# undistro/trivy

Measured on AMD Instinct MI355X. Metric: GB/s secret-scanned (whole node) at 1/2/4/8 MI355X; findings bit-exact vs CPU, higher is better.
Workload: dtype u8

## Files before the change

include/tsg_debug.h:

```cpp
#ifndef TSG_DEBUG_H
#define TSG_DEBUG_H
#include <stdint.h>
#ifdef __cplusplus
extern "C" {
#endif

int tsg_regex_find_all(const char* pattern, const uint8_t* text, uint64_t n, int submatch,
                       const int64_t* windows, uint32_t n_windows, int64_t* out, uint64_t out_cap,
                       uint64_t* out_len, int32_t* num_cap);

void tsg_debug_regex_engine(int mode);
int tsg_debug_xform(int device, const uint8_t* raw, uint64_t n_bytes, const uint64_t* offsets, uint32_t n_files,
                    const uint8_t* kinds, uint8_t* out, uint64_t out_cap, uint64_t* xoff);
int tsg_debug_classify(int device, const uint8_t* raw, uint64_t n_bytes, const uint64_t* offsets, uint32_t n_files,
                       uint8_t* flags);
int tsg_debug_transform_census(int device, const uint8_t* raw, uint64_t n_bytes, const uint64_t* offsets,
                               uint32_t n_files, const uint8_t* kinds, uint8_t* mark_out);
int tsg_debug_gather_device(int device, const uint8_t* raw, uint64_t n_bytes, const uint64_t* src_off,
                            const uint64_t* dst_off, uint32_t n_files, uint8_t* out);
int tsg_regex_match(const char* pattern, const uint8_t* text, uint64_t n);

int64_t tsg_go_bytes_to_lower(const uint8_t* s, uint64_t n, uint8_t* out, uint64_t out_cap);

struct tsg_global;
typedef struct tsg_compiled tsg_compiled;
struct tsg_table_info;
typedef struct tsg_debug_rule_info {
  uint32_t nfa_words;
  uint32_t gate;
  uint32_t anchored;
  uint32_t has_regex;
  const uint64_t* nfa;
  const uint32_t* kw_ids;
  uint32_t n_kw;
} tsg_debug_rule_info;
int tsg_debug_compile(const struct tsg_global* g, tsg_compiled** out);
struct tsg_compile_options;
int tsg_debug_compile_ex(const struct tsg_global* g, const struct tsg_compile_options* opt, tsg_compiled** out,
                         uint32_t* out_calibrated);
void tsg_debug_compiled_free(tsg_compiled* c);
int tsg_debug_compiled_info(const tsg_compiled* c, struct tsg_table_info* out);
int tsg_debug_rule(const tsg_compiled* c, uint32_t i, tsg_debug_rule_info* out);
int tsg_debug_rule_gate_implied(const tsg_compiled* c, uint32_t i);
int tsg_debug_anchor(const tsg_compiled* c, uint32_t j, uint32_t* rule, uint32_t* lit_len,
                     int32_t* off_lo, int32_t* off_hi);
const char* tsg_debug_keyword(const tsg_compiled* c, uint32_t k);
const void* tsg_debug_anchor_req(const tsg_compiled* c, uint32_t j);
int tsg_debug_filter(const tsg_compiled* c, uint32_t* shape, const uint32_t** reach, const uint32_t** bucket_off,
                     const uint32_t** bucket_items, const void** items, uint32_t* n_items, const uint8_t** item_cls,
                     const uint32_t** classes, double* est_fp);
int tsg_debug_filter_ids(const tsg_compiled* c, const uint32_t** ids, uint32_t* n);
const char* tsg_debug_rule_anchor(const tsg_compiled* c, uint32_t i);


int tsg_debug_pool_budget(void);

struct tsg_scanner;
int tsg_debug_scanner_engine(struct tsg_scanner* s, uint64_t out[4]);

int tsg_debug_scanner_gpu_findings(struct tsg_scanner* s, int mode);

int tsg_debug_scanner_fetch(struct tsg_scanner* s, uint64_t stage_bytes, uint64_t direct_bytes);

int tsg_regex_find_all_bounded(const char* pattern, const uint8_t* text, uint64_t true_len, uint64_t lo, uint64_t hi,
                               int submatch, const int64_t* windows, uint32_t n_windows, int64_t* out,
                               uint64_t out_cap, uint64_t* out_len, int32_t* num_cap, int32_t* hit_limit);
int tsg_debug_fetch_windows_plan(const uint64_t* offsets, uint32_t n_files, const void* cands, uint64_t n_cands,
                                 const uint32_t* rule_max_len, uint32_t n_rules, const uint32_t* opts, uint64_t* runs,
                                 uint64_t runs_cap, uint64_t* n_runs, uint64_t* views, uint64_t views_cap,
                                 uint64_t* n_views, uint64_t totals[4]);
int tsg_debug_fetch_windows_device(int device, const uint8_t* arena, uint64_t n_bytes, const uint64_t* offsets,
                                   uint32_t n_files, const void* cands, uint64_t n_cands, uint32_t cand_cap,
                                   const uint32_t* rule_max_len, uint32_t n_rules, const uint32_t* opts,
                                   uint64_t stage_bytes, uint8_t* packed, uint64_t packed_cap, uint64_t counters[4]);

struct tsg_batch;
struct tsg_result;
struct tsg_fetch_window_stats;
int tsg_debug_sparse_tail(const struct tsg_global* g, const struct tsg_batch* batch, const void* cands,
                          uint64_t n_cands, const uint32_t* opts, struct tsg_result** out,
                          struct tsg_fetch_window_stats* window_stats);

int tsg_debug_sure_allow(const char* const* patterns, uint32_t n_patterns, const uint8_t* paths, const uint64_t* off,
                         uint32_t n_paths, uint8_t* sure, uint8_t* has_form);
int tsg_debug_result_skip(const struct tsg_result* r, uint64_t out[6]);
int tsg_debug_result_k0(const struct tsg_result* r, double* ms_k0);

typedef struct tsg_debug_stage_dump {
  uint32_t struct_size;
  uint32_t kw_words;
  uint32_t counters[16];
  uint32_t caps[3];
  uint32_t reserved_;
  uint64_t* hits;        uint64_t hits_cap, n_hits;
  uint32_t* kw;          uint64_t kw_cap, n_kw;
  uint32_t* flags;       uint64_t flags_cap, n_flags;
  uint16_t* nl;          uint64_t nl_cap, n_nl;
  uint32_t* chunk_file;  uint64_t chunk_file_cap, n_chunk_file;
  uint32_t* recs;        uint64_t recs_cap, n_recs;
  void* cands;           uint64_t cands_cap, n_cands;
} tsg_debug_stage_dump;
int tsg_debug_engine_stages(const tsg_compiled* c, int device, const uint8_t* arena, uint64_t n_bytes,
                            const uint64_t* offsets, uint32_t n_files, const uint8_t tail[64],
                            tsg_debug_stage_dump* out);

const char* tsg_last_error(void);

#ifdef __cplusplus
}
#endif
#endif
```

trivy_amd/csrc/capi_debug.cpp:

```cpp
#include "tsg_debug.h"

#include <algorithm>
#include <atomic>
#include <cstring>
#include <memory>
#include <string>
#include <vector>

#include "capi_internal.h"
#include "census.h"
#include "classify.h"
#include "fetch_host.h"
#include "fetch_windows.h"
#include "goregex.h"
#include "parallel.h"
#include "xform.h"

namespace tsg {
extern std::atomic<int> g_regex_engine;
thread_local std::string g_last_error;
void SetError(const std::string& e) { g_last_error = e; }
}

extern "C" {

const char* tsg_last_error(void) { return tsg::g_last_error.c_str(); }

int tsg_regex_find_all(const char* pattern, const uint8_t* text, uint64_t n, int submatch,
                       const int64_t* windows, uint32_t n_windows, int64_t* out, uint64_t out_cap,
                       uint64_t* out_len, int32_t* num_cap) {
  std::string err;
  auto re = tsg::Regex::Compile(pattern, &err);
  if (!re) {
    tsg::SetError(err);
    return -1;
  }
  std::vector<tsg::Window> wins;
  for (uint32_t i = 0; i < n_windows; i++) wins.push_back({windows[2 * i], windows[2 * i + 1]});
  std::vector<int64_t> res;
  re->FindAll(text, int64_t(n), submatch != 0, windows ? &wins : nullptr, &res);
  *out_len = res.size();
  *num_cap = re->num_cap();
  if (!res.empty()) std::memcpy(out, res.data(), sizeof(int64_t) * (res.size() < out_cap ? res.size() : out_cap));
  return 0;
}

void tsg_debug_regex_engine(int mode) { tsg::g_regex_engine.store(mode); }

int tsg_debug_xform(int device, const uint8_t* raw, uint64_t n_bytes, const uint64_t* offsets, uint32_t n_files,
                    const uint8_t* kinds, uint8_t* out, uint64_t out_cap, uint64_t* xoff) {
  if (offsets[0] != 0 || offsets[n_files] != n_bytes) {
    tsg::SetError("offsets must run from 0 to n_bytes");
    return -2;
  }
  void *d_raw = nullptr, *d_off = nullptr, *d_kind = nullptr, *d_xoff = nullptr, *d_out = nullptr, *d_sc = nullptr;
  hipStream_t s = nullptr;
  hipError_t e = hipSetDevice(device);
  auto ok = [&](hipError_t r) {
    if (e == hipSuccess) e = r;
    return e == hipSuccess;
  };
  const size_t sc_bytes = tsg::XformScratchBytes(n_bytes, n_files);
  if (ok(e) && ok(hipStreamCreate(&s)) && ok(hipMalloc(&d_raw, n_bytes + 64)) &&
      ok(hipMalloc(&d_off, (size_t(n_files) + 1) * 8)) && ok(hipMalloc(&d_kind, size_t(n_files) + 1)) &&
      ok(hipMalloc(&d_xoff, (size_t(n_files) + 1) * 8)) && ok(hipMalloc(&d_sc, sc_bytes)) &&
      ok(hipMemset(d_raw, 0, n_bytes + 64)) && ok(hipMemcpy(d_raw, raw, n_bytes, hipMemcpyHostToDevice)) &&
      ok(hipMemcpy(d_off, offsets, (size_t(n_files) + 1) * 8, hipMemcpyHostToDevice)) &&
      ok(hipMemcpy(d_kind, kinds, n_files, hipMemcpyHostToDevice)) && tsg::XformOnePassOn()) {
    const uint64_t cap = tsg::XformMaxOut(n_bytes, n_files) + 64;
    if (ok(hipMalloc(&d_out, cap)) &&
        ok(tsg::XformOnePass(static_cast<const uint8_t*>(d_raw), n_bytes, static_cast<const uint64_t*>(d_off),
                             static_cast<const uint8_t*>(d_kind), n_files, d_sc, static_cast<uint64_t*>(d_xoff),
                             static_cast<uint8_t*>(d_out), cap, s)) &&
        ok(hipMemcpyAsync(xoff, d_xoff, (size_t(n_files) + 1) * 8, hipMemcpyDeviceToHost, s)) &&
        ok(hipStreamSynchronize(s)) &&
        ok(tsg::XformErrorWord(n_bytes, n_files, d_sc, s) == 0 ? hipSuccess : hipErrorIllegalAddress))
      ok(hipMemcpy(out, d_out, std::min<uint64_t>(out_cap, xoff[n_files]), hipMemcpyDeviceToHost));
  } else if (ok(e) &&
      ok(tsg::XformPlan(static_cast<const uint8_t*>(d_raw), n_bytes, static_cast<const uint64_t*>(d_off),
                        static_cast<const uint8_t*>(d_kind), n_files, d_sc, static_cast<uint64_t*>(d_xoff), s)) &&
      ok(hipMemcpyAsync(xoff, d_xoff, (size_t(n_files) + 1) * 8, hipMemcpyDeviceToHost, s)) &&
      ok(hipStreamSynchronize(s)) && ok(hipMalloc(&d_out, xoff[n_files] + 64)) &&
      ok(tsg::XformWrite(static_cast<const uint8_t*>(d_raw), n_bytes, static_cast<const uint64_t*>(d_off),
                         static_cast<const uint8_t*>(d_kind), n_files, d_sc, static_cast<uint8_t*>(d_out),
                         xoff[n_files] + 64, s)) &&
      ok(hipStreamSynchronize(s)) &&
      ok(tsg::XformErrorWord(n_bytes, n_files, d_sc, s) == 0 ? hipSuccess : hipErrorIllegalAddress))
    ok(hipMemcpy(out, d_out, std::min<uint64_t>(out_cap, xoff[n_files]), hipMemcpyDeviceToHost));
  for (void* p : {d_raw, d_off, d_kind, d_xoff, d_out, d_sc})
    if (p) (void)hipFree(p);
  if (s) (void)hipStreamDestroy(s);
  if (e != hipSuccess) {
    tsg::SetError(std::string("tsg_debug_xform: ") + hipGetErrorString(e));
    return -1;
  }
  return 0;
// ... 351 lines not shown
  r->owner = sc.get();
  r->owned = std::move(sc);
  window_stats->mode_used = r->win.mode_used;
  window_stats->granules = r->win.granules;
  window_stats->runs = r->win.runs;
  window_stats->window_bytes = r->win.window_bytes;
  window_stats->sparse_files = r->win.sparse_files;
  window_stats->whole_files = r->win.whole_files;
  window_stats->fallback_files = r->win.fallback_files;
  window_stats->fallback_bytes = r->win.fallback_bytes;
  window_stats->ms_fallback = r->win.ms_fallback;
  *out = r.release();
  return 0;
}

int tsg_debug_engine_stages(const tsg_compiled* c, int device, const uint8_t* arena, uint64_t n_bytes,
                            const uint64_t* offsets, uint32_t n_files, const uint8_t tail[64],
                            tsg_debug_stage_dump* out) {
  if (!c || !offsets || !tail || !out || (n_bytes && !arena)) {
    tsg::SetError("tsg_debug_engine_stages: NULL argument");
    return -2;
  }
  if (out->struct_size != sizeof(tsg_debug_stage_dump)) {
    tsg::SetError("tsg_debug_engine_stages: unknown tsg_debug_stage_dump.struct_size");
    return -2;
  }
  if (!WinArgsOk("tsg_debug_engine_stages", offsets, n_files, nullptr)) return -2;
  if (offsets[n_files] != n_bytes) {
    tsg::SetError("tsg_debug_engine_stages: offsets must end at n_bytes");
    return -2;
  }
  void *d_arena = nullptr, *d_off = nullptr;
  hipError_t e = hipSetDevice(device);
  auto ok = [&](hipError_t r) {
    if (e == hipSuccess) e = r;
    return e == hipSuccess;
  };
  tsg::StageDump d;
  std::string run_err;
  if (ok(e) && ok(hipMalloc(&d_arena, n_bytes + 64)) && ok(hipMalloc(&d_off, (size_t(n_files) + 1) * 8)) &&
      ok(hipMemcpy(static_cast<uint8_t*>(d_arena) + n_bytes, tail, 64, hipMemcpyHostToDevice)) &&
      (n_bytes == 0 || ok(hipMemcpy(d_arena, arena, n_bytes, hipMemcpyHostToDevice))) &&
      ok(hipMemcpy(d_off, offsets, (size_t(n_files) + 1) * 8, hipMemcpyHostToDevice))) {
    std::unique_ptr<tsg::GpuEngine> eng(new tsg::GpuEngine(c->cr, device));
    std::vector<tsg::Candidate> cands;
    if (!eng->ok() || !eng->Run(static_cast<const uint8_t*>(d_arena), n_bytes, static_cast<const uint64_t*>(d_off),
                                n_files, &cands, nullptr, nullptr, nullptr, &d))
      run_err = eng->error().empty() ? "engine failed" : eng->error();
  }
  for (void* p : {d_arena, d_off})
    if (p) (void)hipFree(p);
  if (e != hipSuccess || !run_err.empty()) {
    tsg::SetError(std::string("tsg_debug_engine_stages: ") + (e != hipSuccess ? hipGetErrorString(e) : run_err.c_str()));
    return -1;
  }
  out->kw_words = d.kw_words;
  std::memcpy(out->counters, d.counters, sizeof(out->counters));
  out->caps[0] = d.hit_cap;
  out->caps[1] = d.rec_cap;
  out->caps[2] = d.cand_cap;
  auto put = [](void* dst, uint64_t cap, uint64_t* n, const void* src, size_t count, size_t rec) {
    *n = count;
    const size_t k = size_t(std::min<uint64_t>(cap, count));
    if (dst && k) std::memcpy(dst, src, k * rec);
  };
  std::vector<uint64_t> hits(3 * d.hits.size());
  for (size_t i = 0; i < d.hits.size(); i++) {
    hits[3 * i] = d.hits[i].file;
    hits[3 * i + 1] = d.hits[i].end;
    hits[3 * i + 2] = d.hits[i].aid;
  }
  put(out->hits, out->hits_cap, &out->n_hits, hits.data(), d.hits.size(), 24);
  put(out->kw, out->kw_cap, &out->n_kw, d.kw.data(), d.kw.size(), 4);
  put(out->flags, out->flags_cap, &out->n_flags, d.flags.data(), d.flags.size(), 4);
  put(out->nl, out->nl_cap, &out->n_nl, d.nl.data(), d.nl.size(), 2);
  put(out->chunk_file, out->chunk_file_cap, &out->n_chunk_file, d.chunk_file.data(), d.chunk_file.size(), 4);
  put(out->recs, out->recs_cap, &out->n_recs, d.recs.data(), d.recs.size(), 4);
  put(out->cands, out->cands_cap, &out->n_cands, d.cands.data(), d.cands.size(), sizeof(tsg::Candidate));
  return 0;
}

int tsg_debug_pool_budget(void) { return tsg::PoolBudget(); }

int tsg_debug_sure_allow(const char* const* patterns, uint32_t n_patterns, const uint8_t* paths, const uint64_t* off,
                         uint32_t n_paths, uint8_t* sure, uint8_t* has_form) {
  std::vector<std::unique_ptr<tsg::Regex>> own;
  std::vector<const tsg::Regex*> res;
  for (uint32_t i = 0; i < n_patterns; i++) {
    std::string err;
    own.push_back(tsg::Regex::Compile(patterns[i], &err));
    if (!own.back()) {
      tsg::SetError(err);
      return -1;
    }
    res.push_back(own.back().get());
  }
  tsg::SureTable t;
  std::vector<uint8_t> form;
  tsg::SureTableOf(res, &t, &form);
  if (has_form && n_patterns) std::memcpy(has_form, form.data(), n_patterns);
  for (uint32_t i = 0; i < n_paths; i++) sure[i] = tsg::SureAllowHost(t, paths + off[i], off[i + 1] - off[i]) ? 1 : 0;
  return 0;
}

int tsg_debug_result_skip(const struct tsg_result* r, uint64_t out[6]) {
  if (!r) return -1;
  std::memcpy(out, r->skip, sizeof(r->skip));
  return 0;
}

int tsg_debug_result_k0(const struct tsg_result* r, double* ms_k0) {
  if (!r || !ms_k0) return -1;
  *ms_k0 = r->ms_k0;
  return 0;
}
}
```

trivy_amd/csrc/filter.cpp:

```cpp
#include "filter.h"

#include <algorithm>
#include <cmath>
#include <limits>
#include <cstdlib>
#include <map>

namespace tsg {

const std::vector<double>& BytePrior() {
  static const std::vector<double> prior = [] {
    std::vector<double> f(256, 1e-6);
    static const double en[26] = {8.2, 1.5, 2.8, 4.3, 12.7, 2.2, 2.0, 6.1, 7.0, 0.15, 0.8, 4.0, 2.4,
                                  6.7, 7.5, 1.9, 0.1, 6.0, 6.3, 9.1, 2.8, 1.0, 2.4, 0.15, 2.0, 0.07};
    double tot = 0;
    for (double x : en) tot += x;
    for (int i = 0; i < 26; i++) {
      f['a' + i] = 0.50 * en[i] / tot;
      f['A' + i] = 0.06 * en[i] / tot;
    }
    for (int d = '0'; d <= '9'; d++) f[d] = 0.006;
    for (int c = 0x21; c < 0x7F; c++)
      if (f[c] < 1e-4) f[c] = 0.001;
    f[' '] = 0.14;
    f['\n'] = 0.025;
    f['\t'] = 0.005;
    const std::pair<char, double> punct[] = {{'_', 0.015}, {'.', 0.012}, {',', 0.008}, {'"', 0.01}, {'\'', 0.006},
                                             {'(', 0.008}, {')', 0.008}, {'=', 0.008}, {':', 0.006}, {'-', 0.006},
                                             {'/', 0.005}, {';', 0.004}, {'{', 0.003}, {'}', 0.003}, {'[', 0.002},
                                             {']', 0.002}};
    for (auto& p : punct) f[uint8_t(p.first)] = p.second;
    for (int b = 0x80; b < 0x100; b++) f[b] = 1e-4;
    double s = 0;
    for (double x : f) s += x;
    for (double& x : f) x /= s;
    return f;
  }();
  return prior;
}

namespace {

struct B256 {
  uint64_t w[4];
  void set_all() { w[0] = w[1] = w[2] = w[3] = ~uint64_t(0); }
  bool test(int b) const { return (w[b >> 6] >> (b & 63)) & 1; }
  bool all() const { return (w[0] & w[1] & w[2] & w[3]) == ~uint64_t(0); }
};
B256 ToB256(const ByteSet& s) {
  B256 r{};
  for (int b = 0; b < 256; b++)
    if (s.test(size_t(b))) r.w[b >> 6] |= uint64_t(1) << (b & 63);
  return r;
}

std::vector<double> PriorTable(const std::vector<double>& f) {
  std::vector<double> t(32 * 256, 0.0);
  for (int g = 0; g < 32; g++)
    for (int m = 0; m < 256; m++)
      for (int k = 0; k < 8; k++)
        if ((m >> k) & 1) t[size_t(g) * 256 + size_t(m)] += f[size_t(8 * g + k)];
  return t;
}

thread_local const std::vector<double>* t_prior_table = nullptr;

struct PriorScope {
  std::vector<double> table;
  const std::vector<double>* saved;
  explicit PriorScope(const std::vector<double>* prior) : saved(t_prior_table) {
    if (prior) {
      table = PriorTable(*prior);
      t_prior_table = &table;
    }
  }
  ~PriorScope() { t_prior_table = saved; }
};

double SetProb(const B256& s) {
  static const std::vector<double> T_static = PriorTable(BytePrior());
  const std::vector<double>& T = t_prior_table ? *t_prior_table : T_static;
  if (s.all()) return 1.0;
  double p = 0;
  for (int g = 0; g < 32; g++) p += T[size_t(g) * 256 + ((s.w[g >> 3] >> (8 * (g & 7))) & 0xFF)];
  return std::min(p, 1.0);
}

struct Cluster {
  B256 u[kFilterSlots];
  std::vector<uint32_t> members;
  double cost = 0;
};

constexpr double kRepeatProb = 0.3;
bool SameSingleNonLetter(const B256& a, const B256& b) {
  int n = 0, x = -1;
  for (int k = 0; k < 4; k++) {
    if (a.w[k] != b.w[k]) return false;
    n += __builtin_popcountll(a.w[k]);
    if (a.w[k]) x = 64 * k + __builtin_ctzll(a.w[k]);
  }
  return n == 1 && !((x | 0x20) >= 'a' && (x | 0x20) <= 'z');
}
double WindowProb(const B256* u, int n) {
  double c = 1.0;
  for (int s = 0; s < n; s++) {
    double p = SetProb(u[s]);
    if (s > 0 && SameSingleNonLetter(u[s], u[s - 1])) p = std::max(p, kRepeatProb);
    c *= p;
  }
  return c;
}

double Cost(const B256* u) { return WindowProb(u, kFilterSlots); }

}

void ItemWindow(const FilterItem& it, uint32_t window, size_t* start, size_t* len, const std::vector<double>* prior) {
  PriorScope scope(prior);
  const size_t m = it.sets.size();
  size_t w = 0, wl = std::min<size_t>(m, window);
  double best = std::numeric_limits<double>::infinity();
  for (size_t s = 0; s + wl <= m; s++) {
    B256 win[kFilterSlots];
    for (size_t q = s; q < s + wl; q++) win[q - s] = ToB256(it.sets[q]);
    const double c = WindowProb(win, int(wl));
    if (c < best) {
      best = c;
      w = s;
    }
  }
  *start = w;
  *len = wl;
}

bool BuildFilter(const std::vector<FilterItem>& items, uint32_t window, uint32_t n_buckets, FilterTables* out,
                 std::string* err, const std::vector<double>* prior) {
  PriorScope scope(prior);
  if ((n_buckets != 8 && n_buckets != 16) || window < 2 || window > uint32_t(kFilterSlots)) {
    *err = "unsupported prefilter shape";
    return false;
  }
  *out = FilterTables();
  out->n_buckets = n_buckets;
  out->n_words = n_buckets / 4;
  out->window = window;
  out->nl_bucket = n_buckets - 1;
  const uint32_t n_item_buckets = n_buckets - 1;
  const uint32_t S = window;
  std::vector<FilterItem> uniq;
  std::vector<std::vector<uint32_t>> ids;
  {
    std::map<std::string, size_t> seen;
    for (auto& it : items) {
      std::string key(1, char(it.kind));
      key += char('0' + it.group);
      key += std::to_string(it.lit_end) + ":";
      for (auto& b : it.sets) key += b.to_string();
      auto f = seen.find(key);
      if (f != seen.end() && ids[f->second].size() < 255) {
        ids[f->second].push_back(it.id);
        continue;
      }
      seen[key] = uniq.size();
      uniq.push_back(it);
      ids.push_back({it.id});
    }
  }
  const size_t n = uniq.size();
  std::map<std::string, uint32_t> cls_ids;
  std::vector<ByteSet> classes;
  std::vector<Cluster> cl(n);
  for (size_t i = 0; i < n; i++) {
    const FilterItem& it = uniq[i];
    if (it.sets.empty() || it.sets.size() > 0xFFFF) {
      *err = "prefilter item with no (or too many) positions";
      return false;
    }
    const size_t m = it.sets.size();
    size_t w = 0, wl = 0;
    ItemWindow(it, S, &w, &wl, nullptr);
    for (int s = 0; s < kFilterSlots; s++) cl[i].u[s].set_all();
    for (size_t q = 0; q < wl; q++) cl[i].u[S - wl + q] = ToB256(it.sets[w + q]);
    cl[i].members = {uint32_t(i)};
    cl[i].cost = Cost(cl[i].u);
    FilterItemGpu g{};
    g.n = uint16_t(m);
    g.back = uint16_t(w + wl);
    g.lit_end = uint16_t(it.lit_end);
    g.kind = it.kind;
    g.n_ids = uint8_t(ids[i].size());
    g.ids_off = uint32_t(out->item_ids.size());
    out->item_ids.insert(out->item_ids.end(), ids[i].begin(), ids[i].end());
    g.cls_off = uint32_t(out->item_cls.size());
    out->max_after = std::max<uint32_t>(out->max_after, uint32_t(m - (w + wl)));
    for (auto& b : it.sets) {
      std::string key = b.to_string();
      auto f = cls_ids.find(key);
      uint32_t id;
      if (f == cls_ids.end()) {
        id = uint32_t(classes.size());
        if (id >= 256) {
          *err = "prefilter needs more than 256 distinct byte classes";
          return false;
        }
        cls_ids[key] = id;
        classes.push_back(b);
      } else {
        id = f->second;
      }
      out->item_cls.push_back(uint8_t(id));
    }
    out->items.push_back(g);
  }
  std::vector<bool> alive(n, true);
  size_t n_alive = n;
  auto merged = [&](const Cluster& a, const Cluster& b, B256* u) {
    for (int s = 0; s < kFilterSlots; s++)
      for (int k = 0; k < 4; k++) u[s].w[k] = a.u[s].w[k] | b.u[s].w[k];
    return Cost(u);
  };
  std::vector<bool> solo(n, false);
  if (const char* e = std::getenv("TSG_FILTER_SOLO")) {
    for (const char* q = e; *q;) {
      char* end = nullptr;
      const unsigned long v = std::strtoul(q, &end, 10);
      if (end == q) break;
      if (v < n) solo[v] = true;
      q = *end ? end + 1 : end;
    }
  }
  auto delta_of = [&](size_t i, size_t j) {
    if (solo[i] || solo[j] || uniq[i].group != uniq[j].group) return std::numeric_limits<double>::infinity();
    B256 u[kFilterSlots];
    return merged(cl[i], cl[j], u) - cl[i].cost - cl[j].cost;
  };
  std::vector<double> delta(n > 1 ? n * n : 1, 0.0);
  for (size_t i = 0; i < n; i++)
    for (size_t j = i + 1; j < n; j++) delta[i * n + j] = delta[j * n + i] = delta_of(i, j);
  const double kInf = std::numeric_limits<double>::infinity();
  std::vector<size_t> best(n, 0);
  std::vector<double> best_d(n, kInf);
  auto rescan = [&](size_t i) {
    best_d[i] = kInf;
    for (size_t j = 0; j < n; j++)
      if (j != i && alive[j] && delta[i * n + j] < best_d[i]) {
        best_d[i] = delta[i * n + j];
        best[i] = j;
      }
  };
  for (size_t i = 0; i < n; i++) rescan(i);
  while (n_alive > n_item_buckets) {
    size_t bi = 0, bj = 0;
    double bd = kInf;
    for (size_t i = 0; i < n; i++)
      if (alive[i] && best_d[i] < bd) {
        bd = best_d[i];
        bi = i;
        bj = best[i];
      }
    if (bd == kInf) {
      *err = "prefilter: no bucket merge left (solo items or groups exceed the buckets)";
      return false;
    }
    if (bj < bi) std::swap(bi, bj);
    B256 u[kFilterSlots];
    double c = merged(cl[bi], cl[bj], u);
    for (int s = 0; s < kFilterSlots; s++) cl[bi].u[s] = u[s];
    cl[bi].cost = c;
    cl[bi].members.insert(cl[bi].members.end(), cl[bj].members.begin(), cl[bj].members.end());
    alive[bj] = false;
    n_alive--;
    for (size_t k = 0; k < n; k++) {
      if (!alive[k] || k == bi) continue;
      const double d = delta_of(bi, k);
      delta[k * n + bi] = delta[bi * n + k] = d;
    }
    rescan(bi);
    for (size_t k = 0; k < n; k++) {
      if (!alive[k] || k == bi) continue;
      if (best[k] == bi || best[k] == bj) {
        rescan(k);
      } else if (delta[k * n + bi] < best_d[k]) {
        best_d[k] = delta[k * n + bi];
        best[k] = bi;
      }
    }
  }
  const uint32_t W = out->n_words;
  out->reach.assign(256 * W, ~0u);
  auto allow = [&](uint32_t b, uint32_t j, uint32_t slot) { out->reach[size_t(b) * W + j / 4] &= ~(1u << (4 * slot + j % 4)); };
  out->bucket_off.push_back(0);
  uint32_t j = 0;
  for (size_t i = 0; i < n; i++) {
    if (!alive[i]) continue;
    out->est_fp += cl[i].cost;
    for (uint32_t sl = 0; sl < uint32_t(kFilterSlots); sl++)
      for (int b = 0; b < 256; b++)
        if (sl >= S || cl[i].u[sl].test(b)) allow(uint32_t(b), j, sl);
    for (uint32_t m : cl[i].members) out->bucket_items.push_back(m);
    out->bucket_off.push_back(uint32_t(out->bucket_items.size()));
    j++;
  }
  for (; j < n_buckets; j++) {
    if (j == out->nl_bucket) {
      allow('\n', j, 0);
      for (uint32_t sl = 1; sl < 4; sl++)
        for (int b = 0; b < 256; b++) allow(uint32_t(b), j, sl);
    }
    out->bucket_off.push_back(uint32_t(out->bucket_items.size()));
  }
  std::vector<uint8_t> hashed(n, 0);
  std::vector<std::pair<uint64_t, uint32_t>> hkeys;
  const char* hash_env = std::getenv("TSG_WINDOW_HASH");
  const bool use_hash = hash_env ? std::atoi(hash_env) != 0 && S == 6 : (S == 6 && n > 256);
  for (size_t i = 0; i < n && use_hash; i++) {
    const FilterItemGpu& g = out->items[i];
    if (g.back < 6) continue;
    uint64_t key = 0;
    bool ok = true;
    for (int q = 0; q < 6 && ok; q++) {
      const ByteSet& b = uniq[i].sets[size_t(g.back - 6 + q)];
      const size_t pc = b.count();
      int c = -1;
      for (int x = 0; x < 128 && pc <= 2; x++)
        if (b.test(size_t(x))) {
          c = x;
          break;
        }
      if (c < 0 || pc > 2) {
        ok = false;
        break;
      }
      for (int x = 128; x < 256; x++)
        if (b.test(size_t(x))) ok = false;
// ... 64 lines not shown
```

trivy_amd/csrc/filter.h:

```cpp
#pragma once
#include <cstdint>
#include <string>
#include <vector>

#include "rules.h"

namespace tsg {

constexpr int kFilterSlots = 8;

struct FilterItemGpu {
  uint16_t n;
  uint16_t back;
  uint16_t lit_end;
  uint8_t kind;
  uint8_t n_ids;
  uint32_t ids_off;
  uint32_t cls_off;
};

struct FilterTables {
  uint32_t n_buckets = 0;
  uint32_t n_words = 0;
  uint32_t window = 0;
  uint32_t nl_bucket = 0;
  std::vector<uint32_t> reach;
  std::vector<uint32_t> bucket_off;
  std::vector<uint32_t> bucket_items;
  std::vector<FilterItemGpu> items;
  std::vector<uint32_t> item_ids;
  std::vector<uint8_t> item_cls;
  std::vector<uint32_t> classes;
  std::vector<uint64_t> core;
  std::vector<uint32_t> group_items;
  std::vector<uint32_t> bucket_groups;
  std::vector<uint64_t> hash_keys;
  std::vector<uint32_t> hash_items;
  uint32_t hash_bits = 0;
  uint32_t hash_buckets = 0;
  uint32_t max_after = 0;
  double est_fp = 0;

};

#if defined(__HIPCC__)
#define TSG_HOST_DEVICE __host__ __device__
#else
#define TSG_HOST_DEVICE
#endif
TSG_HOST_DEVICE inline uint32_t WindowHash(uint64_t key, uint32_t bits) {
  return uint32_t((key * 0x9E3779B97F4A7C15ull) >> (64 - bits));
}

const std::vector<double>& BytePrior();

bool BuildFilter(const std::vector<FilterItem>& items, uint32_t window, uint32_t n_buckets, FilterTables* out,
                 std::string* err, const std::vector<double>* prior = nullptr);

void ItemWindow(const FilterItem& it, uint32_t window, size_t* start, size_t* len,
                const std::vector<double>* prior = nullptr);

}
```

trivy_amd/csrc/rules.cpp:

```cpp
#include "rules.h"

#include <cstdio>
#include <cstdlib>

#include "filter.h"

#include <algorithm>
#include <array>
#include <bitset>
#include <deque>
#include <functional>
#include <map>
#include <set>

namespace tsg {

namespace {
constexpr int64_t kInf = int64_t(1) << 40;
constexpr size_t kMaxAnchorLit = 32;

bool IsFoldOnlyRune(uint32_t r) { return r == 0x212A || r == 0x17F || r == 0x130; }

int Utf8Len(uint32_t r) { return r < 0x80 ? 1 : r < 0x800 ? 2 : r < 0x10000 ? 3 : 4; }

// ... 1228 lines not shown
      if (!have) {
        have = class_runs && ExtractClassRun(*re, &best);
      } else if (class_runs && opt && opt->calib && opt->calib_n) {
        Cand run{{}, 0, 0};
        std::vector<std::pair<double, Cand>> runs;
        ExtractClassRun(*re, &run, kClassRunCalibProb, &runs);
        if (!runs.empty()) {
          uint64_t c_lit = 0;
          for (size_t li = 0; li < best.lits.size(); li++)
            c_lit += SampleCost(AnchorItem(*re, best, li, 0), opt->calib, opt->calib_n, cal_prior_p);
          const uint64_t kCalibMinCost = std::max<uint64_t>(16, opt->calib_n / 10000);
          std::sort(runs.begin(), runs.end(), [](const auto& a, const auto& b) { return a.first < b.first; });
          if (runs.size() > 4) runs.resize(4);
          for (auto& cr : runs) {
            if (c_lit < kCalibMinCost) break;
            const uint64_t c_run = SampleCost(AnchorItem(*re, cr.second, 0, 0), opt->calib, opt->calib_n, cal_prior_p);
            if (std::getenv("TSG_CALIB_DEBUG"))
              std::fprintf(stderr, "calib %s: literal %llu, class run of %zu at [%lld,%lld] %llu\n", r.id.c_str(),
                           (unsigned long long)c_lit, cr.second.lits[0].size(), (long long)cr.second.olo,
                           (long long)cr.second.ohi, (unsigned long long)c_run);
            if (2 * c_run < c_lit) {
              best = cr.second;
              c_lit = c_run;
              calibrated = true;
            }
          }
          if (calibrated) out->n_calibrated_anchors++;
        }
      }
      if (have) {
        rg.anchored = 1;
        desc = "[" + std::to_string(best.olo) + "," + std::to_string(best.ohi) + "]";
        if (calibrated) desc += " (calibrated)";
        for (size_t li = 0; li < best.lits.size(); li++) {
          const std::string& l = best.lits[li];
          uint32_t aid = uint32_t(out->anchors.size());
          AnchorInfo ai{};
          ai.rule = uint32_t(ri);
          ai.lit_len = uint32_t(l.size());
          ai.off_lo = int32_t(best.olo);
          ai.off_hi = int32_t(best.ohi);
          ai.off_hi_fold = int32_t(std::min<int64_t>(best.ohi_fold, 1 << 30));
          out->anchors.push_back(ai);
          out->anchor_req.push_back(FollowReqs(re->nodes(), best.follow[li]));
          out->items.push_back(AnchorItem(*re, best, li, aid));
          if (calibrated) out->items.back().group = 1;
          desc += best.class_run ? " <" + std::to_string(l.size()) + " classes>" : " " + l;
        }
      } else {
        rg.anchored = 0;
        out->n_fullscan_rules++;
      }
      {
        const int64_t mx = Analyzer(re->nodes(), true).Bytes(re->root()).second;
        const int64_t mn = Analyzer(re->nodes(), false).Bytes(re->root()).first;
        rg.min_len = uint32_t(std::min<int64_t>(std::max<int64_t>(mn, 0), 1 << 30));
        rg.max_len = mx >= (int64_t(1) << 20) ? kNoMaxLen : uint32_t(mx);
      }
      BuildNfa(Relax(re->nodes(), re->root()), &out->nfa, &rg);
    }
    out->rule_anchor_desc.push_back(desc);
    out->rules.push_back(rg);
    out->regex.push_back(std::move(re));
  }
  {
    const char* seqs[3] = {"\xC4\xB0", "\xE2\x84\xAA", "\xC5\xBF"};
    for (uint32_t k = 0; k < 3; k++) {
      FilterItem fi;
      fi.kind = kItemFold;
      fi.id = k;
      for (const char* p = seqs[k]; *p; p++) {
        ByteSet b;
        b.set(uint8_t(*p));
        fi.sets.push_back(b);
      }
      fi.lit_end = uint32_t(fi.sets.size());
      out->items.push_back(std::move(fi));
    }
  }
  {
    uint32_t nb = 16, nw = FilterWindow();
    if (const char* e = std::getenv("TSG_FILTER_BUCKETS")) nb = uint32_t(std::atoi(e));
    auto ft = std::make_shared<FilterTables>();
    if (!BuildFilter(out->items, nw, nb, ft.get(), err, cal_prior_p)) return false;
    out->filter = ft;
  }
  return true;
}

}
```

Measured before the change: 2607.

## Build prefilter buckets by measuring false-fire rates on a calibration sample

When a calibration sample is provided and no calibrated prior is set, the prefilter bucket assignment comes from a measured objective instead of the prior-based greedy merge. For each item, bitset columns over a prefix of the sample give the actual fire count per candidate window. Items are then merged greedily and refined with moves, window changes and swaps. The goal is fewer false prefilter hits, and so less downstream regex verification work. The cost is extra compile time, and the path is used only when opt->calib is supplied and the prior path is unused.

```diff
diff --git a/include/tsg_debug.h b/include/tsg_debug.h
--- a/include/tsg_debug.h
+++ b/include/tsg_debug.h
@@ -50,6 +50,7 @@
                      const uint32_t** bucket_items, const void** items, uint32_t* n_items, const uint8_t** item_cls,
                      const uint32_t** classes, double* est_fp);
 int tsg_debug_filter_ids(const tsg_compiled* c, const uint32_t** ids, uint32_t* n);
+int tsg_debug_filter_core(const tsg_compiled* c, uint32_t out[4]);
 const char* tsg_debug_rule_anchor(const tsg_compiled* c, uint32_t i);
 
 
diff --git a/trivy_amd/csrc/capi_debug.cpp b/trivy_amd/csrc/capi_debug.cpp
--- a/trivy_amd/csrc/capi_debug.cpp
+++ b/trivy_amd/csrc/capi_debug.cpp
@@ -12,6 +12,7 @@
 #include "classify.h"
 #include "fetch_host.h"
 #include "fetch_windows.h"
+#include "filter.h"
 #include "goregex.h"
 #include "parallel.h"
 #include "xform.h"
@@ -529,6 +530,25 @@
 
 int tsg_debug_pool_budget(void) { return tsg::PoolBudget(); }
 
+int tsg_debug_filter_core(const tsg_compiled* c, uint32_t out[4]) {
+  const auto* f = c->cr.filter.get();
+  if (!f) return -1;
+  const uint32_t n_groups = uint32_t(f->core.size() / 256);
+  std::vector<std::vector<uint64_t>> cols;
+  for (uint32_t b = 0; b < 256; b++) {
+    std::vector<uint64_t> col(n_groups);
+    for (uint32_t g = 0; g < n_groups; g++) col[g] = f->core[size_t(g) * 256 + b];
+    if (std::find(cols.begin(), cols.end(), col) == cols.end()) cols.push_back(std::move(col));
+  }
+  uint32_t most = 0;
+  for (uint32_t b = 0; b + 1 < f->bucket_groups.size(); b++) most = std::max(most, f->bucket_groups[b + 1] - f->bucket_groups[b]);
+  out[0] = n_groups;
+  out[1] = uint32_t(cols.size());
+  out[2] = most;
+  out[3] = uint32_t(f->hash_keys.size());
+  return 0;
+}
+
 int tsg_debug_sure_allow(const char* const* patterns, uint32_t n_patterns, const uint8_t* paths, const uint64_t* off,
                          uint32_t n_paths, uint8_t* sure, uint8_t* has_form) {
   std::vector<std::unique_ptr<tsg::Regex>> own;
diff --git a/trivy_amd/csrc/filter.cpp b/trivy_amd/csrc/filter.cpp
--- a/trivy_amd/csrc/filter.cpp
+++ b/trivy_amd/csrc/filter.cpp
@@ -1,10 +1,15 @@
 #include "filter.h"
 
 #include <algorithm>
+#include <chrono>
+#include <cstdio>
 #include <cmath>
 #include <limits>
 #include <cstdlib>
+#include <functional>
 #include <map>
+
+#include "parallel.h"
 
 namespace tsg {
 
@@ -77,13 +82,15 @@
   ~PriorScope() { t_prior_table = saved; }
 };
 
-double SetProb(const B256& s) {
-  static const std::vector<double> T_static = PriorTable(BytePrior());
-  const std::vector<double>& T = t_prior_table ? *t_prior_table : T_static;
+double SetProbT(const B256& s, const std::vector<double>& T) {
   if (s.all()) return 1.0;
   double p = 0;
   for (int g = 0; g < 32; g++) p += T[size_t(g) * 256 + ((s.w[g >> 3] >> (8 * (g & 7))) & 0xFF)];
   return std::min(p, 1.0);
+}
+double SetProb(const B256& s) {
+  static const std::vector<double> T_static = PriorTable(BytePrior());
+  return SetProbT(s, t_prior_table ? *t_prior_table : T_static);
 }
 
 struct Cluster {
@@ -113,6 +120,468 @@
 }
 
 double Cost(const B256* u) { return WindowProb(u, kFilterSlots); }
+
+constexpr uint64_t kCalibPrefixBytes = 2u << 20;
+constexpr double kCalibLambda = 0.03;
+using Col = std::vector<uint64_t>;
+struct SlotCol {
+  const uint64_t* p;
+  unsigned sh;
+};
+inline uint64_t Ld(const SlotCol& c, size_t w) {
+  return c.sh ? (c.p[w] << c.sh) | (w ? c.p[w - 1] >> (64 - c.sh) : 0) : c.p[w];
+}
+constexpr size_t kColBlock = 256;
+inline const uint64_t* LdBlock(const SlotCol& c, size_t w0, size_t cnt, uint64_t* buf) {
+  if (!c.sh) return c.p + w0;
+  size_t k = 0;
+  if (w0 == 0) {
+    buf[0] = c.p[0] << c.sh;
+    k = 1;
+  }
+  const unsigned sh = c.sh, rs = 64 - c.sh;
+  const uint64_t* p = c.p + w0;
+  for (; k < cnt; k++) buf[k] = (p[k] << sh) | (p[k - 1] >> rs);
+  return buf;
+}
+inline uint64_t PopBlock(const uint64_t* v, size_t cnt) {
+  uint64_t n = 0;
+  for (size_t k = 0; k < cnt; k++) n += uint64_t(__builtin_popcountll(v[k]));
+  return n;
+}
+
+struct Win {
+  size_t start = 0, len = 0;
+  SlotCol c[kFilterSlots];
+  B256 u[kFilterSlots];
+};
+
+struct Calib {
+  uint32_t S = 0;
+  size_t words = 0;
+  double n_pos = 0, lambda = 0;
+  std::vector<double> ptab;
+  std::vector<Col> base;
+  std::vector<B256> cls_set;
+  Col ones;
+  int threads = 1;
+  bool static_reg = false;
+
+  double Reg(const B256* u) const {
+    if (static_reg) return lambda * n_pos * WindowProb(u, int(S));
+    double p = lambda * n_pos;
+    for (uint32_t s = 0; s < S; s++) p *= SetProbT(u[s], ptab);
+    return p;
+  }
+  static double Groups(size_t k) { return double((k + 7) / 8); }
+  double Obj(uint64_t fires, const B256* u, size_t k) const { return (double(fires) + Reg(u)) * Groups(k); }
+
+  Win MakeWin(const uint8_t* cls, size_t start, size_t len) const {
+    Win w;
+    w.start = start;
+    w.len = len;
+    for (int s = 0; s < kFilterSlots; s++) {
+      w.c[s] = {ones.data(), 0};
+      w.u[s].set_all();
+    }
+    for (size_t q = 0; q < len; q++) {
+      const size_t sl = S - len + q;
+      w.c[sl] = {base[cls[start + q]].data(), unsigned(S - 1 - sl)};
+      w.u[sl] = cls_set[cls[start + q]];
+    }
+    return w;
+  }
+  uint64_t Fires(const SlotCol* a) const {
+    uint64_t n = 0, acc[kColBlock], bx[kColBlock];
+    for (size_t w0 = 0; w0 < words; w0 += kColBlock) {
+      const size_t cnt = std::min(kColBlock, words - w0);
+      for (size_t k = 0; k < cnt; k++) acc[k] = ~uint64_t(0);
+      for (uint32_t s = 0; s < S; s++) {
+        const uint64_t* x = LdBlock(a[s], w0, cnt, bx);
+        for (size_t k = 0; k < cnt; k++) acc[k] &= x[k];
+      }
+      n += PopBlock(acc, cnt);
+    }
+    return n;
+  }
+  uint64_t PairFires(const SlotCol* a, const SlotCol* b) const {
+    uint64_t n = 0, acc[kColBlock], bx[kColBlock], by[kColBlock];
+    for (size_t w0 = 0; w0 < words; w0 += kColBlock) {
+      const size_t cnt = std::min(kColBlock, words - w0);
+      for (size_t k = 0; k < cnt; k++) acc[k] = ~uint64_t(0);
+      for (uint32_t s = 0; s < S; s++) {
+        const uint64_t* x = LdBlock(a[s], w0, cnt, bx);
+        const uint64_t* y = LdBlock(b[s], w0, cnt, by);
+        for (size_t k = 0; k < cnt; k++) acc[k] &= x[k] | y[k];
+      }
+      n += PopBlock(acc, cnt);
+    }
+    return n;
+  }
+};
+
+struct MCluster {
+  SlotCol c[kFilterSlots];
+  std::vector<Col> own;
+  B256 u[kFilterSlots];
+  std::vector<uint32_t> members;
+  double obj = 0;
+};
+
+struct MBucket {
+  std::vector<uint32_t> members;
+  std::vector<Col> U, U2;
+  double obj = 0;
+};
+
+uint64_t FiresRemAdd(const Calib& C, const MBucket& b, const Win* rem, const Win* add) {
+  uint64_t n = 0, acc[kColBlock], bx[kColBlock], by[kColBlock];
+  for (size_t w0 = 0; w0 < C.words; w0 += kColBlock) {
+    const size_t cnt = std::min(kColBlock, C.words - w0);
+    for (size_t k = 0; k < cnt; k++) acc[k] = ~uint64_t(0);
+    for (uint32_t s = 0; s < C.S; s++) {
+      const uint64_t* U = b.U[s].data() + w0;
+      const uint64_t* U2 = b.U2[s].data() + w0;
+      const uint64_t* x = rem ? LdBlock(rem->c[s], w0, cnt, bx) : nullptr;
+      const uint64_t* y = add ? LdBlock(add->c[s], w0, cnt, by) : nullptr;
+      if (x && y) {
+        for (size_t k = 0; k < cnt; k++) acc[k] &= U2[k] | (U[k] & ~x[k]) | y[k];
+      } else if (x) {
+        for (size_t k = 0; k < cnt; k++) acc[k] &= U2[k] | (U[k] & ~x[k]);
+      } else if (y) {
+        for (size_t k = 0; k < cnt; k++) acc[k] &= U[k] | y[k];
+      } else {
+        for (size_t k = 0; k < cnt; k++) acc[k] &= U[k];
+      }
+    }
+    n += PopBlock(acc, cnt);
+  }
+  return n;
+}
+double ObjRemAdd(const Calib& C, const std::vector<Win>& win, const MBucket& b, int64_t rem, const Win* add) {
+  B256 u[kFilterSlots] = {};
+  size_t k = 0;
+  for (uint32_t m : b.members) {
+    if (int64_t(m) == rem) continue;
+    k++;
+    for (uint32_t s = 0; s < C.S; s++)
+      for (int q = 0; q < 4; q++) u[s].w[q] |= win[m].u[s].w[q];
+  }
+  if (add) {
+    k++;
+    for (uint32_t s = 0; s < C.S; s++)
+      for (int q = 0; q < 4; q++) u[s].w[q] |= add->u[s].w[q];
+  }
+  if (k == 0) return 0;
+  return C.Obj(FiresRemAdd(C, b, rem >= 0 ? &win[size_t(rem)] : nullptr, add), u, k);
+}
+void Rebuild(const Calib& C, const std::vector<Win>& win, MBucket* b) {
+  b->U.assign(C.S, Col(C.words, 0));
+  b->U2.assign(C.S, Col(C.words, 0));
+  for (uint32_t m : b->members)
+    for (uint32_t s = 0; s < C.S; s++) {
+      uint64_t* U = b->U[s].data();
+      uint64_t* U2 = b->U2[s].data();
+      for (size_t w = 0; w < C.words; w++) {
+        const uint64_t x = Ld(win[m].c[s], w);
+        U2[w] |= U[w] & x;
+        U[w] |= x;
+      }
+    }
+  b->obj = ObjRemAdd(C, win, *b, -1, nullptr);
+}
+
+void MeasuredBuckets(const std::vector<FilterItem>& uniq, const std::vector<uint8_t>& item_cls,
+                     const std::vector<uint32_t>& cls_off, const std::vector<ByteSet>& classes, uint32_t S,
+                     uint32_t n_item_buckets, const uint8_t* sample, uint64_t sample_n,
+                     const std::function<bool(size_t, size_t)>& may_share, const std::vector<bool>& fixed,
+                     std::vector<size_t>* wstart, std::vector<size_t>* wlen, std::vector<std::vector<uint32_t>>* buckets) {
+  const size_t n = uniq.size();
+  Calib C;
+  C.S = S;
+  const bool debug = std::getenv("TSG_CALIB_DEBUG") != nullptr;
+  auto t0 = std::chrono::steady_clock::now();
+  auto lap = [&](const char* what) {
+    if (!debug) return;
+    const auto t1 = std::chrono::steady_clock::now();
+    std::fprintf(stderr, "calib buckets: %s %.3f s\n", what, std::chrono::duration<double>(t1 - t0).count());
+    t0 = t1;
+  };
+  uint64_t prefix = kCalibPrefixBytes;
+  if (const char* e = std::getenv("TSG_CALIB_PREFIX_KB")) prefix = uint64_t(std::atoll(e)) << 10;
+  const uint64_t N = std::min<uint64_t>(sample_n, std::max<uint64_t>(prefix, 64));
+  C.words = size_t((N + 63) / 64);
+  C.n_pos = double(N);
+  C.lambda = kCalibLambda;
+  if (const char* e = std::getenv("TSG_CALIB_LAMBDA")) C.lambda = std::atof(e);
+  if (const char* e = std::getenv("TSG_CALIB_REG")) C.static_reg = std::atoi(e) == 1;
+  C.threads = 16;
+  if (const char* e = std::getenv("TSG_COMPILE_THREADS")) C.threads = std::max(1, std::atoi(e));
+  {
+    std::vector<uint64_t> h(256, 0);
+    for (uint64_t i = 0; i < sample_n; i++) h[sample[i]]++;
+    const double K = 65536.0;
+    std::vector<double> f(256);
+    for (int b = 0; b < 256; b++) f[size_t(b)] = (double(h[size_t(b)]) + K * BytePrior()[size_t(b)]) / (double(sample_n) + K);
+    C.ptab = PriorTable(f);
+  }
+  C.ones.assign(C.words, ~uint64_t(0));
+  C.base.assign(classes.size(), Col());
+  C.cls_set.resize(classes.size());
+  ParallelFor(classes.size(), C.threads, [&](size_t k) {
+    C.cls_set[k] = ToB256(classes[k]);
+    uint8_t in[256];
+    for (int b = 0; b < 256; b++) in[b] = classes[k].test(size_t(b)) ? 1 : 0;
+    Col& col = C.base[k];
+    col.assign(C.words, 0);
+    for (uint64_t t = 0; t < N; t++) col[size_t(t >> 6)] |= uint64_t(in[sample[t]]) << (t & 63);
+  });
+  lap("columns");
+  const bool measure_windows = !std::getenv("TSG_CALIB_WINDOWS") || std::atoi(std::getenv("TSG_CALIB_WINDOWS")) != 0;
+  std::vector<Win> win(n);
+  std::vector<std::vector<Win>> cands(n);
+  ParallelFor(n, C.threads, [&](size_t i) {
+    const uint8_t* cls = item_cls.data() + cls_off[i];
+    const size_t m = uniq[i].sets.size(), wl = (*wlen)[i];
+    win[i] = C.MakeWin(cls, (*wstart)[i], wl);
+    if (!measure_windows) return;
+    double best = C.Obj(C.Fires(win[i].c), win[i].u, 1);
+    for (size_t s = 0; s + wl <= m; s++) {
+      cands[i].push_back(C.MakeWin(cls, s, wl));
+      if (s == (*wstart)[i]) continue;
+      const double o = C.Obj(C.Fires(cands[i].back().c), cands[i].back().u, 1);
+      if (o < best) {
+        best = o;
+        win[i] = cands[i].back();
+      }
+    }
+  });
+  lap("windows");
+  std::vector<MCluster> mc(n);
+  for (size_t i = 0; i < n; i++) {
+    for (int s = 0; s < kFilterSlots; s++) {
+      mc[i].c[s] = win[i].c[s];
+      mc[i].u[s] = win[i].u[s];
+    }
+    mc[i].members = {uint32_t(i)};
+  }
+  ParallelFor(n, C.threads, [&](size_t i) { mc[i].obj = C.Obj(C.Fires(mc[i].c), mc[i].u, 1); });
+  const double kInf = std::numeric_limits<double>::infinity();
+  std::vector<bool> alive(n, true);
+  auto cluster_ok = [&](size_t i, size_t j) {
+    for (uint32_t a : mc[i].members)
+      for (uint32_t b : mc[j].members)
+        if (fixed[a] || fixed[b] || !may_share(a, b)) return false;
+    return true;
+  };
+  auto delta_of = [&](size_t i, size_t j) {
+    if (!cluster_ok(i, j)) return kInf;
+    B256 u[kFilterSlots];
+    for (int s = 0; s < kFilterSlots; s++)
+      for (int k = 0; k < 4; k++) u[s].w[k] = mc[i].u[s].w[k] | mc[j].u[s].w[k];
+    return C.Obj(C.PairFires(mc[i].c, mc[j].c), u, mc[i].members.size() + mc[j].members.size()) - mc[i].obj - mc[j].obj;
+  };
+  std::vector<double> delta(n > 1 ? n * n : 1, 0.0);
+  ParallelFor(n, C.threads, [&](size_t i) {
+    for (size_t j = i + 1; j < n; j++) delta[i * n + j] = delta_of(i, j);
+  });
+  for (size_t i = 0; i < n; i++)
+    for (size_t j = i + 1; j < n; j++) delta[j * n + i] = delta[i * n + j];
+  size_t n_alive = n;
+  while (n_alive > n_item_buckets) {
+    size_t bi = 0, bj = 0;
+    double bd = kInf;
+    for (size_t i = 0; i < n; i++)
+      for (size_t j = i + 1; j < n; j++)
+        if (alive[i] && alive[j] && delta[i * n + j] < bd) {
+          bd = delta[i * n + j];
+          bi = i;
+          bj = j;
+        }
+    if (bd == kInf) break;
+    std::vector<Col> own(S, Col(C.words));
+    for (uint32_t s = 0; s < S; s++)
+      for (size_t w = 0; w < C.words; w++) own[s][w] = Ld(mc[bi].c[s], w) | Ld(mc[bj].c[s], w);
+    mc[bi].own.swap(own);
+    for (uint32_t s = 0; s < S; s++) {
+      mc[bi].c[s] = {mc[bi].own[s].data(), 0};
+      for (int k = 0; k < 4; k++) mc[bi].u[s].w[k] |= mc[bj].u[s].w[k];
+    }
+    mc[bi].members.insert(mc[bi].members.end(), mc[bj].members.begin(), mc[bj].members.end());
+    mc[bi].obj = C.Obj(C.Fires(mc[bi].c), mc[bi].u, mc[bi].members.size());
+    mc[bj].own.clear();
+    alive[bj] = false;
+    n_alive--;
+    ParallelFor(n, C.threads, [&](size_t k) {
+      if (!alive[k] || k == bi) return;
+      delta[k * n + bi] = delta[bi * n + k] = delta_of(bi, k);
+    });
+  }
+  lap("greedy");
+  std::vector<MBucket> bk;
+  std::vector<uint32_t> bof(n, 0);
+  for (size_t i = 0; i < n; i++)
+    if (alive[i]) {
+      for (uint32_t m : mc[i].members) bof[m] = uint32_t(bk.size());
+      bk.emplace_back();
+      bk.back().members = mc[i].members;
+    }
+  mc.clear();
+  ParallelFor(bk.size(), C.threads, [&](size_t b) { Rebuild(C, win, &bk[b]); });
+  struct Change {
+    double d = 0;
+    uint32_t x = 0, y = 0xFFFFFFFFu, to = 0;
+    size_t cand = size_t(-1);
+  };
+  const bool refine = !std::getenv("TSG_CALIB_REFINE") || std::atoi(std::getenv("TSG_CALIB_REFINE")) != 0;
+  bool windows_done = !measure_windows;
+  auto movable = [&](size_t x, size_t b) {
+    if (fixed[x]) return false;
+    for (uint32_t m : bk[b].members)
+      if (m != x && (fixed[m] || !may_share(x, m))) return false;
+    return true;
+  };
+  std::vector<double> mcost(n * bk.size(), 0.0), mgain(n, 0.0);
+  std::vector<uint32_t> mcost_v(n * bk.size(), 0), mgain_v(n, 0);
+  std::vector<uint32_t> bver(bk.size(), 1), sw_b(n, 0xFFFFFFFFu), sw_va(n, 0), sw_vb(n, 0);
+  std::vector<Change> sw_ch(n);
+  int n_rounds = 0, n_changes[3] = {0, 0, 0};
+  for (int round = 0; refine && round < 400; round++) {
+    n_rounds++;
+    double total = 0;
+    for (auto& b : bk) total += b.obj;
+    const double eps = 1e-9 * (total + 1.0);
+    std::vector<Change> ch(n);
+    std::vector<uint32_t> pref(n, 0xFFFFFFFFu);
+    auto apply = [&](int phase) {
+      std::vector<size_t> order;
+      for (size_t i = 0; i < n; i++)
+        if (ch[i].d < -eps) order.push_back(i);
+      std::sort(order.begin(), order.end(), [&](size_t a, size_t b) { return ch[a].d != ch[b].d ? ch[a].d < ch[b].d : a < b; });
+      std::vector<bool> touched(bk.size(), false);
+      std::vector<size_t> dirty;
+      for (size_t i : order) {
+        const Change& c = ch[i];
+        const uint32_t A = bof[c.x], B = phase == 1 ? A : c.to;
+        if (touched[A] || touched[B]) continue;
+        touched[A] = touched[B] = true;
+        bver[A]++;
+        if (B != A) bver[B]++;
+        n_changes[phase]++;
+        dirty.push_back(A);
+        if (phase == 1) {
+          for (size_t b = 0; b < bk.size(); b++) mcost_v[c.x * bk.size() + b] = 0;
+          win[c.x] = cands[c.x][c.cand];
+          continue;
+        }
+        dirty.push_back(B);
+        auto& ma = bk[A].members;
+        ma.erase(std::find(ma.begin(), ma.end(), c.x));
+        bk[B].members.push_back(c.x);
+        bof[c.x] = B;
+        if (phase == 2) {
+          auto& mb = bk[B].members;
+          mb.erase(std::find(mb.begin(), mb.end(), c.y));
+          ma.push_back(c.y);
+          bof[c.y] = A;
+        }
+      }
+      ParallelFor(dirty.size(), C.threads, [&](size_t k) { Rebuild(C, win, &bk[dirty[k]]); });
+      return !dirty.empty();
+    };
+    ParallelFor(n, C.threads, [&](size_t x) {
+      const uint32_t A = bof[x];
+      if (fixed[x] || bk[A].members.size() < 2) return;
+      if (mgain_v[x] != bver[A]) {
+        mgain[x] = bk[A].obj - ObjRemAdd(C, win, bk[A], int64_t(x), nullptr);
+        mgain_v[x] = bver[A];
+      }
+      const double gain = mgain[x];
+      double best = kInf;
+      for (uint32_t B = 0; B < bk.size(); B++) {
+        if (B == A || !movable(x, B)) continue;
+        if (mcost_v[x * bk.size() + B] != bver[B]) {
+          mcost[x * bk.size() + B] = ObjRemAdd(C, win, bk[B], -1, &win[x]) - bk[B].obj;
+          mcost_v[x * bk.size() + B] = bver[B];
+        }
+        const double cost = mcost[x * bk.size() + B];
+        if (cost < best) {
+          best = cost;
+          pref[x] = B;
+        }
+      }
+      if (pref[x] != 0xFFFFFFFFu) {
+        ch[x].d = best - gain;
+        ch[x].x = uint32_t(x);
+        ch[x].to = pref[x];
+      }
+    });
+    if (apply(0)) continue;
+    if (!windows_done) {
+      windows_done = true;
+      ch.assign(n, Change());
+      ParallelFor(n, C.threads, [&](size_t x) {
+        const MBucket& A = bk[bof[x]];
+        for (size_t k = 0; k < cands[x].size(); k++) {
+          if (cands[x][k].start == win[x].start) continue;
+          const double d = ObjRemAdd(C, win, A, int64_t(x), &cands[x][k]) - A.obj;
+          if (d < ch[x].d) {
+            ch[x].d = d;
+            ch[x].x = uint32_t(x);
+            ch[x].cand = k;
+          }
+        }
+      });
+      if (apply(1)) continue;
+    }
+    ch.assign(n, Change());
+    ParallelFor(n, C.threads, [&](size_t x) {
+      const uint32_t A = bof[x], B = pref[x];
+      if (B == 0xFFFFFFFFu) return;
+      if (sw_b[x] == B && sw_va[x] == bver[A] && sw_vb[x] == bver[B]) {
+        ch[x] = sw_ch[x];
+        return;
+      }
+      sw_b[x] = B;
+      sw_va[x] = bver[A];
+      sw_vb[x] = bver[B];
+      sw_ch[x] = Change();
+      for (uint32_t y : bk[B].members) {
+        if (fixed[y]) continue;
+        bool ok = true;
+        for (uint32_t m : bk[A].members)
+          if (m != x && !may_share(y, m)) ok = false;
+        for (uint32_t m : bk[B].members)
+          if (m != y && !may_share(x, m)) ok = false;
+        if (!ok) continue;
+        const double d = ObjRemAdd(C, win, bk[A], int64_t(x), &win[y]) + ObjRemAdd(C, win, bk[B], int64_t(y), &win[x]) -
+                         bk[A].obj - bk[B].obj;
+        if (d < ch[x].d) {
+          ch[x].d = d;
+          ch[x].x = uint32_t(x);
+          ch[x].y = y;
+          ch[x].to = B;
+        }
+      }
+      sw_ch[x] = ch[x];
+    });
+    if (!apply(2)) break;
+  }
+  lap("refinement");
+  if (debug)
+    std::fprintf(stderr, "calib buckets: %d rounds, %d moves, %d windows, %d swaps\n", n_rounds, n_changes[0], n_changes[1],
+                 n_changes[2]);
+  for (size_t i = 0; i < n; i++) {
+    (*wstart)[i] = win[i].start;
+    (*wlen)[i] = win[i].len;
+  }
+  buckets->clear();
+  for (auto& b : bk) {
+    std::sort(b.members.begin(), b.members.end());
+    buckets->push_back(b.members);
+  }
+  std::sort(buckets->begin(), buckets->end());
+}
 
 }
 
@@ -135,7 +604,7 @@
 }
 
 bool BuildFilter(const std::vector<FilterItem>& items, uint32_t window, uint32_t n_buckets, FilterTables* out,
-                 std::string* err, const std::vector<double>* prior) {
+                 std::string* err, const std::vector<double>* prior, const uint8_t* sample, uint64_t sample_n) {
   PriorScope scope(prior);
   if ((n_buckets != 8 && n_buckets != 16) || window < 2 || window > uint32_t(kFilterSlots)) {
     *err = "unsupported prefilter shape";
@@ -171,6 +640,8 @@
   std::map<std::string, uint32_t> cls_ids;
   std::vector<ByteSet> classes;
   std::vector<Cluster> cl(n);
+  std::vector<size_t> wstart(n, 0), wlen(n, 0);
+  std::vector<uint32_t> cls_off(n, 0);
   for (size_t i = 0; i < n; i++) {
     const FilterItem& it = uniq[i];
     if (it.sets.empty() || it.sets.size() > 0xFFFF) {
@@ -180,6 +651,9 @@
     const size_t m = it.sets.size();
     size_t w = 0, wl = 0;
     ItemWindow(it, S, &w, &wl, nullptr);
+    wstart[i] = w;
+    wlen[i] = wl;
+    cls_off[i] = uint32_t(out->item_cls.size());
     for (int s = 0; s < kFilterSlots; s++) cl[i].u[s].set_all();
     for (size_t q = 0; q < wl; q++) cl[i].u[S - wl + q] = ToB256(it.sets[w + q]);
     cl[i].members = {uint32_t(i)};
@@ -250,7 +724,39 @@
       }
   };
   for (size_t i = 0; i < n; i++) rescan(i);
-  while (n_alive > n_item_buckets) {
+  const bool measured = sample && sample_n >= 4096 && n <= 256;
+  if (measured) {
+    std::vector<std::vector<uint32_t>> buckets;
+    const char* ge = std::getenv("TSG_CALIB_GROUPS");
+    const bool keep_groups = ge && std::atoi(ge) != 0;
+    MeasuredBuckets(uniq, out->item_cls, cls_off, classes, S, n_item_buckets, sample, sample_n,
+                    [&](size_t a, size_t b) { return !keep_groups || uniq[a].group == uniq[b].group; }, solo, &wstart,
+                    &wlen, &buckets);
+    if (buckets.size() > n_item_buckets) {
+      *err = "prefilter: no bucket merge left (solo items or groups exceed the buckets)";
+      return false;
+    }
+    out->max_after = 0;
+    for (size_t i = 0; i < n; i++) {
+      alive[i] = false;
+      const size_t m = uniq[i].sets.size(), w = wstart[i], wl = wlen[i];
+      for (int s = 0; s < kFilterSlots; s++) cl[i].u[s].set_all();
+      for (size_t q = 0; q < wl; q++) cl[i].u[S - wl + q] = ToB256(uniq[i].sets[w + q]);
+      out->items[i].back = uint16_t(w + wl);
+      out->max_after = std::max<uint32_t>(out->max_after, uint32_t(m - (w + wl)));
+    }
+    for (auto& b : buckets) {
+      Cluster& c = cl[b[0]];
+      for (size_t k = 1; k < b.size(); k++)
+        for (int s = 0; s < kFilterSlots; s++)
+          for (int q = 0; q < 4; q++) c.u[s].w[q] |= cl[b[k]].u[s].w[q];
+      c.members = b;
+      c.cost = Cost(c.u);
+      alive[b[0]] = true;
+    }
+    n_alive = buckets.size();
+  }
+  while (!measured && n_alive > n_item_buckets) {
     size_t bi = 0, bj = 0;
     double bd = kInf;
     for (size_t i = 0; i < n; i++)
diff --git a/trivy_amd/csrc/filter.h b/trivy_amd/csrc/filter.h
--- a/trivy_amd/csrc/filter.h
+++ b/trivy_amd/csrc/filter.h
@@ -55,7 +55,8 @@
 const std::vector<double>& BytePrior();
 
 bool BuildFilter(const std::vector<FilterItem>& items, uint32_t window, uint32_t n_buckets, FilterTables* out,
-                 std::string* err, const std::vector<double>* prior = nullptr);
+                 std::string* err, const std::vector<double>* prior = nullptr, const uint8_t* sample = nullptr,
+                 uint64_t sample_n = 0);
 
 void ItemWindow(const FilterItem& it, uint32_t window, size_t* start, size_t* len,
                 const std::vector<double>* prior = nullptr);
diff --git a/trivy_amd/csrc/rules.cpp b/trivy_amd/csrc/rules.cpp
--- a/trivy_amd/csrc/rules.cpp
+++ b/trivy_amd/csrc/rules.cpp
@@ -1334,7 +1334,11 @@
     uint32_t nb = 16, nw = FilterWindow();
     if (const char* e = std::getenv("TSG_FILTER_BUCKETS")) nb = uint32_t(std::atoi(e));
     auto ft = std::make_shared<FilterTables>();
-    if (!BuildFilter(out->items, nw, nb, ft.get(), err, cal_prior_p)) return false;
+    const char* cb_env = std::getenv("TSG_CALIB_BUCKETS");
+    const bool by_sample = opt && opt->calib && opt->calib_n && !cal_prior_p && !(cb_env && std::atoi(cb_env) == 0);
+    if (!BuildFilter(out->items, nw, nb, ft.get(), err, cal_prior_p, by_sample ? opt->calib : nullptr,
+                     by_sample ? opt->calib_n : 0))
+      return false;
     out->filter = ft;
   }
   return true;
```

Result: faster. 2835 (median of 6 runs) (+8.8%).
